# ultravideo/uvg266

Hardware: AMD Instinct MI355X
Metric: encoded fps (1080p all-intra --preset medium closed loop: CTU search with the reference's RD decisions -> deblock -> SAO -> slice data; Mpixels/s in config) (higher is better)
Workload: dtype u8

## Files before the change

### uvg266_amd/csrc/ctu_core.h

```cpp
#pragma once
#include <stdint.h>
#include <stddef.h>
#include <string.h>
#include "intra_pred_dev.h"
#if defined(__HIPCC__)
#include "satd_dev.h"
#endif
#include "vvc_tables.h"
#include "vvc_ctx_init.h"
#include "vvc_rdoq_tables.h"
#include "../../include/uvg266_hip.h"
#if defined(CTU_PB)
#include "inter_cand_dev.h"
#endif

#if defined(__HIPCC__)
#define CTU_NOINLINE __attribute__((noinline))
#define CTU_INLINE __attribute__((always_inline))
#define CTU_INLINE1 __attribute__((always_inline))
#define CTU_DEV static __device__
#define CTU_SHARED __shared__
#define CTU_TID ((int)(threadIdx.x & 63))
#define CTU_NT 64
#define CTU_WAVE (__builtin_amdgcn_readfirstlane((int)((threadIdx.x >> 6) - S->rot) & 3))
// ... 244 lines not shown
#if !defined(CTU_PB)
  int32_t req64, done64[2], m64[2];
  int32_t creq, cdone[2];
  struct { int32_t cu, cv, ssd_u, ssd_v, cy, ssd_y; double bits, bits_y; } h64[4];
#endif
  alignas(16) unsigned char arena[lds_cfg<PX>::slim ? (int)ARENA_BYTES_SLIM : (int)ARENA_BYTES];
#if defined(CTU_PB)
  pb_state pb;
  int32_t leaf_wave;
  double leaf_cost[4];
  double leaf_limit;
  int32_t depth_wave, skip_eval[4];
  pb_state pbx;
  alignas(16) unsigned char arena8[arena_bytes(8)];
  alignas(16) int16_t b8_tmp[6 * 2 * 120];
  PX b8_pred[6 * 64];
  int32_t b8_satd[8];
  pb_state pbx2;
  alignas(16) unsigned char arena16[arena_bytes(16)];
  alignas(16) PX cand64_px[6144];
  int16_t cand64_co[6144];
  uint32_t cur64[NMX];
#endif
};
#if defined(CTU_PB)
template <typename PX> constexpr size_t pb_lds_bytes(int waves) { return waves >= 4 ? sizeof(lds<PX>) : (waves == 3 ? offsetof(lds<PX>, pbx2) : offsetof(lds<PX>, pbx)); }
template <typename PX> CTU_DEV pb_state &pbq(lds<PX> *S) { const int r = CTU_WAVE; return r == 2 ? S->pbx : (r == 3 ? S->pbx2 : S->pb); }
#endif
template <typename PX> CTU_DEV wctx *wv_of(lds<PX> *S) { return &S->wv[S->vsel[CTU_WAVE]]; }

struct scratch {
  double cost_coeff[1024], cost_sig[1024], cost_coeff0[1024];
  uint16_t save_px[6144];
  int16_t save_co[6144];
  cu4 save_cu[256];
  int16_t cand_co[2016];
  uint16_t cand_px32[1536];
  int16_t lv32[1536];
  uint16_t scan_g[1024 + 256];
  uint32_t save_tree[512];
  uint16_t tree[256], mtt[256];
#if defined(CTU_PB)
  int32_t save_mot[256][8];
  uint8_t save_fl[256][8];
  int32_t pb_mot[17 * 17 + 1][8];
  uint8_t pb_fl[17 * 17][8];
  unsigned long long prof_pb[24];
#endif
  unsigned long long prof_lf[16];
  unsigned long long prof[4][32];
};

template <typename PX> struct job {
  params P;
  const PX *src_y, *src_u, *src_v;
  int src_stride, src_stride_c;
  PX *rec_y, *rec_u, *rec_v;
  int rec_stride, rec_stride_c;
  uvghip_scu_t *cu_tab;
  int cu_stride;
  int16_t *coeff;
  uint32_t *models_out;
  const uint32_t *models_in;
  scratch *W;
  int x, y;
#if defined(CTU_PB)
  const struct pb_job *pb;
  uint32_t *pbm_out;
  const uint32_t *pbm_in;
  int slice_type, init_qp;
#endif
};

template <typename PX> CTU_DEV CTU_GLB const PX *src_block(const job<PX> &J, int color, int bx, int by, int *pitch)
{
  const PX *p = color == 0 ? J.src_y : (color == 1 ? J.src_u : J.src_v);
  const int st = color == 0 ? J.src_stride : J.src_stride_c, sh = color != 0;
  *pitch = st;
  return (CTU_GLB const PX *)(p + (size_t)((J.y >> sh) + by) * st + (J.x >> sh) + bx);
}


CTU_DEV uint32_t *tab_ebits() { CTU_SHARED uint32_t t[512]; return t; }
CTU_DEV uint8_t *tab_rate() { CTU_SHARED uint8_t t[(NMX + 7) & ~7]; return t; }
CTU_DEV uint32_t *tab_rdoq_bits() { CTU_SHARED uint32_t t[2 * 244]; return t; }
#define kRate (tab_rate())

template <typename MP> CTU_DEV int m_state(MP m, int c) { return (int)(((m[c] & 0xffffu) + (m[c] >> 16)) >> 8); }
template <typename MP> CTU_DEV void m_update(MP m, int c, int bin)
{
  const int r0 = kRate[c] >> 4, r1 = kRate[c] & 15;
  uint32_t s0 = m[c] & 0xffffu, s1 = m[c] >> 16;
  s0 -= (s0 >> r0) & 0x7fe0u;
  s1 -= (s1 >> r1) & 0x7ffeu;
  if (bin) { s0 += (0x7fffu >> r0) & 0x7fe0u; s1 += (0x7fffu >> r1) & 0x7ffeu; }
  m[c] = (s0 & 0xffffu) | (s1 << 16);
}
template <typename MP> CTU_DEV double m_fbits(MP m, int c, int bin) { return (double)tab_ebits()[(m_state(m, c) << 1) ^ bin] / 32768.0; }
template <typename MP> CTU_DEV void m_code(MP m, int update, int c, int bin, double &bits)
{
  bits += m_fbits(m, c, bin);
  if (update) m_update(m, c, bin);
}

CTU_DEV void models_init_one(uint32_t *m, int i, int qp, int slice)
{
  const int v = k_ctx_init[slice][i];
  if (v == 255) { m[i] = 0; return; }
  const int slope = (v >> 3) - 4, offset = ((v & 7) * 18) + 1;
  int s = ((slope * (qp - 16)) >> 1) + offset;
  s = s < 1 ? 1 : (s > 127 ? 127 : s);
  const uint32_t p1 = (uint32_t)s << 8;
  m[i] = (p1 & 0x7fe0u) | ((p1 & 0x7ffeu) << 16);
}

CTU_DEV int scan_base(int log2n) { return log2n == 5 ? 0 : log2n == 4 ? 1024 : log2n == 3 ? 1280 : 1344; }
template <typename PX> CTU_DEV uint16_t *scan_of(lds<PX> *S, int log2n)
{
  if (lds_cfg<PX>::slim_scan) return log2n >= 4 ? S->scr->scan_g + (log2n == 5 ? 0 : 1024) : S->scan + (log2n == 3 ? 0 : 64);
  return S->scan + scan_base(log2n);
}
CTU_DEV int last_bits_off(int t, int log2n, int xy)
{
  const int cnt = 2 * log2n;
  const int base = log2n == 2 ? 0 : (log2n == 3 ? 8 : (log2n == 4 ? 20 : 36));
  return (t ? 56 : 0) + base + (xy ? cnt : 0);
}
CTU_DEV void diag_order(int n, uint8_t *out)
{
  int i = 0;
  for (int d = 0; d < 2 * n - 1; ++d)
    for (int x = 0; x <= d; ++x) {
      const int y = d - x;
      if (x < n && y < n) out[i++] = (uint8_t)(y * n + x);
    }
}
CTU_DEV int rdoq_diag_start(int n, int d)
{
  return d < n ? d * (d + 1) / 2 : n * n - (2 * n - 1 - d) * (2 * n - d) / 2;
}
template <typename PX> CTU_DEV void build_scans(lds<PX> *S)
{
  SERIAL {
    uint8_t in[16], cg[64];
    diag_order(4, in);
    for (int l2 = 2; l2 <= 5; ++l2) {
      const int n = 1 << l2, cgw = n >> 2;
      diag_order(cgw, cg);
      uint16_t *sc = scan_of(S, l2);
      if (l2 == 2) {
        for (int k = 0; k < 16; ++k) S->inv4[in[k]] = (uint8_t)k;
        for (int k = 0; k < 16; ++k) {
          const int x = in[k] & 3, y = in[k] >> 2;
          unsigned m = 0;
          if (x + 1 < 4) m |= 1u << S->inv4[y * 4 + x + 1];
          if (x + 2 < 4) m |= 1u << S->inv4[y * 4 + x + 2];
          if (y + 1 < 4) m |= 1u << S->inv4[(y + 1) * 4 + x];
          if (y + 2 < 4) m |= 1u << S->inv4[(y + 2) * 4 + x];
          if (x + 1 < 4 && y + 1 < 4) m |= 1u << S->inv4[(y + 1) * 4 + x + 1];
          S->deps4[k] = (uint16_t)m;
        }
      }
      for (int g = 0; g < cgw * cgw; ++g) {
        const int gx = cg[g] % cgw, gy = cg[g] / cgw;
        for (int k = 0; k < 16; ++k) sc[g * 16 + k] = (uint16_t)((gy * 4 + in[k] / 4) * n + gx * 4 + in[k] % 4);
      }
    }
  }
  CTU_SYNC();
}

CTU_DEV int16_t *lv_of(wctx *V, int color) { return color == 0 ? V->lv0 : (color == 1 ? V->lv1 : V->lv2); }
template <typename PX> CTU_DEV PX *plane(lds<PX> *S, int color) { return color == 0 ? S->Dy : (color == 1 ? S->Du : S->Dv); }
CTU_DEV int pitch_of(int color) { return color == 0 ? PY : PC; }
template <typename PX> CTU_DEV cu4 *cu_at(lds<PX> *S, int lx, int ly) { return &S->cu[((ly >> 2) + 1) * 17 + (lx >> 2) + 1]; }

template <typename PX> CTU_DEV int count_edge_cus(lds<PX> *S, int x, int y, int lx, int ly, int n, int left)
{
  if ((left && x == 0) || (!left && y == 0)) return 0;
  if (left && lx == 0) return (LCU - ly) / 4;
  if (!left && ly == 0) return n / 2;
  int amount = n & ~3;
  if (left) {
    if (ly == 0 && lx == 32 && cu_at(S, lx, ly)->log2 == 6) return 8;
    while (ly + amount < LCU && cu_at(S, lx - 4, ly + amount)->type != CU_NOTSET) amount += 4;
  } else {
    while (lx + amount < LCU && cu_at(S, lx + amount, ly - 4)->type != CU_NOTSET) amount += 4;
  }
  return (amount / 4) > (n / 4) ? amount / 4 : n / 4;
}

template <typename PX> CTU_NOINLINE CTU_DEV void build_refs(lds<PX> *S, const params &P, int color, int x, int y, int lx, int ly, int n, int cu_n)
{
  wctx *const V = wv_of(S);
  const int c = color != 0;
  const int w = n >> c;
  const int px_x = lx >> c, px_y = ly >> c;
  const int pit = pitch_of(color);
  const PX *D = plane(S, color) + (px_y + 1) * pit + px_x + 1;
  SERIAL {
    int al = count_edge_cus(S, x, y, lx, ly, n, 1) * (c ? 2 : 4);
    if (al > 2 * w) al = 2 * w;
    if (al > ((P.pic_h - y) >> c)) al = (P.pic_h - y) >> c;
    int at = count_edge_cus(S, x, y, lx, ly, n, 0) * (c ? 2 : 4);
    if (at > 2 * w) at = 2 * w;
    if (at > ((P.pic_w - x) >> c)) at = (P.pic_w - x) >> c;
    if (x > 0 && y > 0 && P.wpp && px_y == 0 && at > (LCU >> c) - px_x) at = (LCU >> c) - px_x;
    V->u_avail_left = al; V->u_avail_top = at;
  }
  CTU_SYNC();
  const int al = V->u_avail_left, at = V->u_avail_top;
  const int dc = 1 << (px_info<PX>::depth - 1);
  CTU_LDS uint16_t *const r_top = LDSP(uint16_t, V->top), *const r_left = LDSP(uint16_t, V->left);
  CTU_LDS uint16_t *const r_ftop = LDSP(uint16_t, V->ftop), *const r_fleft = LDSP(uint16_t, V->fleft);
  PAR_FOR(i, V->refn - 1) {
    int lv, tv;
    if (x > 0) lv = D[(i < al ? i : al - 1) * pit - 1];
    else lv = y > 0 ? D[-pit] : dc;
    if (y > 0) tv = D[-pit + (i < at ? i : at - 1)];
    else tv = x > 0 ? D[-1] : dc;
    r_left[i + 1] = (uint16_t)lv;
    r_top[i + 1] = (uint16_t)tv;
  }
  SERIAL {
    int corner;
    if (x > 0 && y > 0) corner = D[-pit - 1];
    else corner = x > 0 ? D[-1] : (y > 0 ? D[-pit] : dc);
    r_left[0] = r_top[0] = (uint16_t)corner;
  }
  CTU_SYNC();
  const int flim = 2 * (cu_n >> c) < V->refn - 1 ? 2 * (cu_n >> c) : V->refn - 1;
  PAR_FOR(i, V->refn) {
    int fl, ft;
    if (i == 0) fl = ft = (r_left[1] + 2 * r_left[0] + r_top[1] + 2) >> 2;
    else {
      fl = i < flim ? (r_left[i - 1] + 2 * r_left[i] + r_left[i + 1] + 2) >> 2 : r_left[i];
      ft = i < flim ? (r_top[i - 1] + 2 * r_top[i] + r_top[i + 1] + 2) >> 2 : r_top[i];
    }
    r_fleft[i] = (uint16_t)fl;
    r_ftop[i] = (uint16_t)ft;
  }
  CTU_SYNC();
}

template <typename PX> CTU_NOINLINE CTU_DEV void predict_block(lds<PX> *S, int mode, int color, int w, PX *dst_, int dp)
{
  wctx *const V = wv_of(S);
  const mode_info M = make_mode_info(mode, w, w, color != 0);
  const ref_rows_t<CTU_LDS const uint16_t *> R = {LDSP(const uint16_t, V->top), LDSP(const uint16_t, V->left), LDSP(const uint16_t, V->ftop), LDSP(const uint16_t, V->fleft)};
  const int dc = mode == 1 ? dc_value(R.top, R.left, w, w) : 0;
  typename mg_ptr<PX, PX>::type const dst = MGP(PX, PX, dst_);
  const int segs = w >> 2;
  PAR_FOR(t, w * segs) {
    const int yd = t / segs, xd0 = (t - yd * segs) * 4;
    int out[4];
    predict_row<4>(M, R, dc, color != 0, w, w, yd, xd0, (int)px_info<PX>::maxv, out);
    for (int i = 0; i < 4; ++i) {
      const int bx = M.vertical ? xd0 + i : yd, by = M.vertical ? yd : xd0 + i;
      dst[by * dp + bx] = (PX)out[i];
    }
  }
  CTU_SYNC();
}

CTU_DEV int iabs_(int v) { return v < 0 ? -v : v; }
CTU_DEV unsigned satd8_tile(int (&d)[64])
{
  for (int pass = 0; pass < 2; ++pass) {
    const int s = pass ? 8 : 1, t = pass ? 1 : 8;
    for (int l = 0; l < 8; ++l) {
      int *v = &d[l * t];
      for (int half = 4; half >= 1; half >>= 1)
        for (int base = 0; base < 8; base += 2 * half)
          for (int i = 0; i < half; ++i) {
            const int p = v[(base + i) * s], q = v[(base + i + half) * s];
            v[(base + i) * s] = p + q;
            v[(base + i + half) * s] = p - q;
          }
    }
  }
  unsigned sad = 0;
  for (int i = 0; i < 64; ++i) sad += (unsigned)iabs_(d[i]);
  sad -= (unsigned)iabs_(d[0]);
  sad += (unsigned)iabs_(d[0]) >> 2;
  return (sad + 2) >> 2;
}
CTU_DEV unsigned satd4_tile(int (&d)[16])
{
  for (int pass = 0; pass < 2; ++pass) {
    const int s = pass ? 4 : 1, t = pass ? 1 : 4;
    for (int l = 0; l < 4; ++l) {
      int *v = &d[l * t];
      const int a = v[0] + v[2 * s], b = v[0] - v[2 * s], c2 = v[s] + v[3 * s], e = v[s] - v[3 * s];
      v[0] = a + c2; v[s] = a - c2; v[2 * s] = b + e; v[3 * s] = b - e;
    }
  }
  unsigned satd = 0;
  for (int i = 0; i < 16; ++i) satd += (unsigned)iabs_(d[i]);
  satd -= (unsigned)iabs_(d[0]);
  satd += (unsigned)iabs_(d[0]) >> 2;
  return (satd + 1) >> 1;
}

template <typename PX> CTU_NOINLINE CTU_DEV void rough_costs(lds<PX> *S, const job<PX> &J, int lx, int ly, int n, const int32_t *modes, int n_modes)
{
  wctx *const V = wv_of(S);
  int sps;
  CTU_GLB const PX *Sy = src_block(J, 0, lx, ly, &sps);
  const int T = n >= 8 ? 8 : 4, tiles_x = n / T, tiles = tiles_x * tiles_x;
  const ref_rows_t<CTU_LDS const uint16_t *> R = {LDSP(const uint16_t, V->top), LDSP(const uint16_t, V->left), LDSP(const uint16_t, V->ftop), LDSP(const uint16_t, V->fleft)};
  const int dcv = dc_value(R.top, R.left, n, n);
  CTU_LDS uint32_t *const part = LDSP(uint32_t, V->part);
#if defined(__HIPCC__)
  const int n_flat = (n_modes > 0 && modes[0] < 2) + (n_modes > 1 && modes[1] < 2);
  for (int seg = 0; seg < 2; ++seg) {
  const int m_first = seg ? 0 : n_flat, total = (seg ? n_flat : n_modes - n_flat) * tiles * T;
  for (int base = 0; base < total; base += CTU_NT) {
    const int idx = base + CTU_TID;
    const bool on = idx < total;
    const int task0 = on ? idx / T : 0, r = idx & (T - 1);
    const int task = task0 + m_first * tiles;
    const int mi = task / tiles, tile = task - mi * tiles;
    const mode_info M = make_mode_info(modes[mi], n, n, 0);
    const int ty = tile / tiles_x, tx = tile - ty * tiles_x;
    int sad = 0, satd;
    if (T == 8) {
      int d[8], out[8];
      predict_row<8>(M, R, dcv, 0, n, n, ty * 8 + r, tx * 8, (int)px_info<PX>::maxv, out);
#pragma unroll
      for (int i = 0; i < 8; ++i) {
        const int wx = tx * 8 + i, wy = ty * 8 + r;
        const int bx = M.vertical ? wx : wy, by = M.vertical ? wy : wx;
        d[i] = on ? (int)Sy[by * sps + bx] - out[i] : 0;
        sad += iabs_(d[i]);
      }
      satd = satd8_cost(d, r);
      sad = dpp_group_sum<8>(sad);
    } else {
      int d[4], out[4];
      predict_row<4>(M, R, dcv, 0, n, n, r, 0, (int)px_info<PX>::maxv, out);
#pragma unroll
      for (int i = 0; i < 4; ++i) {
        const int bx = M.vertical ? i : r, by = M.vertical ? r : i;
        d[i] = on ? (int)Sy[by * sps + bx] - out[i] : 0;
        sad += iabs_(d[i]);
      }
      satd = satd4_cost(d, r);
      sad = dpp_group_sum<4>(sad);
    }
    if (on && r == 0) { part[2 * task] = (uint32_t)satd; part[2 * task + 1] = (uint32_t)sad; }
  }
  }
  CTU_SYNC();
#else
  PAR_FOR(task, n_modes * tiles) {
    const int mi = task / tiles, tile = task - mi * tiles;
    const int mode = modes[mi];
    const mode_info M = make_mode_info(mode, n, n, 0);
    const int ty = tile / tiles_x, tx = tile - ty * tiles_x;
    unsigned sad = 0, satd;
    if (T == 8) {
      int d[64];
      for (int r = 0; r < 8; ++r) {
        int out[8];
        predict_row<8>(M, R, dcv, 0, n, n, ty * 8 + r, tx * 8, (int)px_info<PX>::maxv, out);
        for (int i = 0; i < 8; ++i) {
          const int wx = tx * 8 + i, wy = ty * 8 + r;
          const int bx = M.vertical ? wx : wy, by = M.vertical ? wy : wx;
          const int df = (int)Sy[by * sps + bx] - out[i];
          d[r * 8 + i] = df;
          sad += (unsigned)iabs_(df);
        }
      }
      satd = satd8_tile(d);
    } else {
      int d[16];
      for (int r = 0; r < 4; ++r) {
        int out[4];
        predict_row<4>(M, R, dcv, 0, n, n, r, 0, (int)px_info<PX>::maxv, out);
        for (int i = 0; i < 4; ++i) {
          const int bx = M.vertical ? i : r, by = M.vertical ? r : i;
          const int df = (int)Sy[by * sps + bx] - out[i];
          d[r * 4 + i] = df;
          sad += (unsigned)iabs_(df);
        }
      }
      satd = satd4_tile(d);
    }
    part[2 * task] = satd;
    part[2 * task + 1] = sad;
  }
  CTU_SYNC();
#endif
}

#if defined(__HIPCC__)
CTU_DEV uint64_t rs_key(double c) { return (uint64_t)(uint32_t)__double2hiint(c) << 32 | (uint32_t)__double2loint(c); }
CTU_DEV uint32_t rs_wave_min(uint32_t v)
{
#define RS_MIN(x) { const uint32_t o = (uint32_t)(x); v = o < v ? o : v; }
  RS_MIN(__builtin_amdgcn_update_dpp(0, (int)v, 0xB1, 0xf, 0xf, true));
  RS_MIN(__builtin_amdgcn_update_dpp(0, (int)v, 0x4E, 0xf, 0xf, true));
  RS_MIN(__builtin_amdgcn_update_dpp(0, (int)v, 0x141, 0xf, 0xf, true));
  RS_MIN(__builtin_amdgcn_update_dpp(0, (int)v, 0x140, 0xf, 0xf, true));
  RS_MIN(__builtin_amdgcn_update_dpp((int)v, (int)v, 0x142, 0xa, 0xf, false));
  RS_MIN(__builtin_amdgcn_update_dpp((int)v, (int)v, 0x143, 0xc, 0xf, false));
#undef RS_MIN
  return (uint32_t)__builtin_amdgcn_readlane((int)v, 63);
}
struct rs_extra { bool on; uint64_t key; int seq, mode; };
struct rs_pick { int who; uint64_t key; };
CTU_DEV bool rs_key_lt(uint32_t khi, uint32_t klo, uint64_t k) { return ((uint64_t)khi << 32 | klo) < k; }
template <bool X> CTU_DEV rs_pick rs_pick_min(bool on, uint32_t khi, uint32_t klo, int seq, const rs_extra &x)
{
  const uint32_t none = 0xffffffffu;
  const uint32_t xh = (uint32_t)(x.key >> 32), xl = (uint32_t)x.key;
  const bool xon = X && x.on;
  rs_pick r;
  const unsigned long long b_on = __ballot(on);
  const int n_on = __popcll(b_on) + (xon ? 1 : 0);
  if (n_on == 0) { r.who = 0; r.key = ~0ull; return r; }
  uint32_t mh = 0;
  unsigned long long b1 = b_on;
  bool y = xon;
  if (n_on > 1) {
    mh = rs_wave_min(on ? khi : none);
    if (xon && xh < mh) mh = xh;
    b1 = __ballot(on && khi == mh);
    y = xon && xh == mh;
  }
  if (__popcll(b1) + (y ? 1 : 0) == 1) {
    if (y) { r.who = 64; r.key = x.key; }
    else {
      r.who = __builtin_ctzll(b1);
      r.key = (uint64_t)(uint32_t)__builtin_amdgcn_readlane((int)khi, r.who) << 32 | (uint32_t)__builtin_amdgcn_readlane((int)klo, r.who);
    }
    return r;
  }
  const bool t1 = on && khi == mh;
  uint32_t ml = rs_wave_min(t1 ? klo : none);
  if (y && xl < ml) ml = xl;
  const bool t2 = t1 && klo == ml, z = y && xl == ml;
  uint32_t ms = rs_wave_min(t2 ? (uint32_t)seq : none);
  r.key = (uint64_t)mh << 32 | ml;
  if (z && (uint32_t)x.seq < ms) r.who = 64;
  else {
    const unsigned long long w = __ballot(t2 && (uint32_t)seq == ms);
    r.who = w ? __builtin_ctzll(w) : 0;
  }
  return r;
}
struct rs_top3 { int m[3]; uint64_t k[3]; };
CTU_DEV void rs_insert(rs_top3 &B, int mode, uint64_t key)
{
  if (key < B.k[0]) { B.k[2] = B.k[1]; B.m[2] = B.m[1]; B.k[1] = B.k[0]; B.m[1] = B.m[0]; B.k[0] = key; B.m[0] = mode; }
  else if (key < B.k[1]) { B.k[2] = B.k[1]; B.m[2] = B.m[1]; B.k[1] = key; B.m[1] = mode; }
  else if (key < B.k[2]) { B.k[2] = key; B.m[2] = mode; }
}
template <bool X> CTU_DEV void rs_round(rs_top3 &B, bool on, uint32_t khi, uint32_t klo, int seq, int mode, rs_extra x)
{
  for (int i = 0; i < 3; ++i) {
    on = on && rs_key_lt(khi, klo, B.k[2]);
    if (X) x.on = x.on && x.key < B.k[2];
    const rs_pick pk = rs_pick_min<X>(on, khi, klo, seq, x);
    if (pk.key == ~0ull) break;
    rs_insert(B, pk.who < 64 ? __builtin_amdgcn_readlane(mode, pk.who) : x.mode, pk.key);
    on = on && CTU_TID != pk.who;
    if (X) x.on = x.on && pk.who != 64;
  }
}
#endif

CTU_DEV double count_bits(const int8_t *preds, double planar, double not_planar, double mpm_bit, double not_mpm_bit, int mode)
{
  int i = 0, smaller = 0;
  for (; i < 6; i++) {
    if (preds[i] == mode) break;
    if (mode > preds[i]) smaller += 1;
  }
  if (i == 0) return planar + mpm_bit;
  if (i < 6) return not_planar + mpm_bit + (i < 4 ? i : 4);
  return not_mpm_bit + 5 + (mode - smaller > 2);
}

CTU_DEV void dir_luma_predictor(int y, int8_t *preds, const cu4 *left_pu, const cu4 *above_pu)
{
  int left_dir = 0, above_dir = 0;
  if (left_pu && left_pu->type == CU_INTRA) left_dir = left_pu->mode;
  if (above_pu && above_pu->type == CU_INTRA && y % LCU != 0) above_dir = above_pu->mode;
  const int offset = 61, mod = 64;
  preds[0] = 0; preds[1] = 1; preds[2] = 50; preds[3] = 18; preds[4] = 46; preds[5] = 54;
  if (left_dir == above_dir) {
    if (left_dir > 1) {
      preds[0] = 0; preds[1] = (int8_t)left_dir;
      preds[2] = (int8_t)(((left_dir + offset) % mod) + 2); preds[3] = (int8_t)(((left_dir - 1) % mod) + 2);
      preds[4] = (int8_t)(((left_dir + offset - 1) % mod) + 2); preds[5] = (int8_t)((left_dir % mod) + 2);
    }
  } else if (left_dir > 1 && above_dir > 1) {
    preds[0] = 0; preds[1] = (int8_t)left_dir; preds[2] = (int8_t)above_dir;
    const int mx = preds[1] > preds[2] ? 1 : 2, mn = preds[1] > preds[2] ? 2 : 1;
    const int diff = preds[mx] - preds[mn];
    if (diff == 1) {
      preds[3] = (int8_t)(((preds[mn] + offset) % mod) + 2); preds[4] = (int8_t)(((preds[mx] - 1) % mod) + 2);
      preds[5] = (int8_t)(((preds[mn] + offset - 1) % mod) + 2);
    } else if (diff >= 62) {
      preds[3] = (int8_t)(((preds[mn] - 1) % mod) + 2); preds[4] = (int8_t)(((preds[mx] + offset) % mod) + 2);
      preds[5] = (int8_t)((preds[mn] % mod) + 2);
    } else if (diff == 2) {
      preds[3] = (int8_t)(((preds[mn] - 1) % mod) + 2); preds[4] = (int8_t)(((preds[mn] + offset) % mod) + 2);
      preds[5] = (int8_t)(((preds[mx] - 1) % mod) + 2);
    } else {
      preds[3] = (int8_t)(((preds[mn] + offset) % mod) + 2); preds[4] = (int8_t)(((preds[mn] - 1) % mod) + 2);
      preds[5] = (int8_t)(((preds[mx] + offset) % mod) + 2);
    }
  } else if (left_dir + above_dir >= 2) {
    preds[0] = 0;
    preds[1] = (int8_t)(left_dir < above_dir ? above_dir : left_dir);
    preds[2] = (int8_t)(((preds[1] + offset) % mod) + 2); preds[3] = (int8_t)(((preds[1] - 1) % mod) + 2);
    preds[4] = (int8_t)(((preds[1] + offset - 1) % mod) + 2); preds[5] = (int8_t)((preds[1] % mod) + 2);
  }
}
template <typename PX> CTU_DEV void mpm_neighbours(lds<PX> *S, int x, int y, int lx, int ly, int n, const cu4 **left, const cu4 **above)
{
  *left = x > 0 ? cu_at(S, lx - 1, ly + n - 1) : nullptr;
  *above = (ly > 0 && y > 0) ? cu_at(S, lx + n - 1, ly - 1) : nullptr;
}

#if defined(__HIPCC__)
template <typename PX> CTU_INLINE1 CTU_DEV void search_intra_rough(lds<PX> *S, const job<PX> &J, int x, int y, int lx, int ly, int n)
{
  wctx *const V = wv_of(S);
  const params &P = J.P;
  const int T = n >= 8 ? 8 : 4, tiles = (n / T) * (n / T);
  const int lane = CTU_TID;
  RQ_T0(J.W)
  SERIAL {
    const cu4 *l, *a;
    mpm_neighbours(S, x, y, lx, ly, n, &l, &a);
    dir_luma_predictor(y, V->mpm, l, a);
  }
  int offset = 1 << __builtin_amdgcn_readfirstlane(P.rough_levels);
  const int first_m = 2 + offset / 2;
  int nm = 2 + (66 - first_m) / offset + 1;
  if (lane < nm) V->rs_list[lane] = lane < 2 ? lane : first_m + (lane - 2) * offset;
  uint32_t pat = 1u << (first_m & (offset - 1));
  for (int sh = offset; sh < 32; sh <<= 1) pat |= pat << sh;
  uint32_t h0 = (pat & ~((1u << first_m) - 1u)) | 3u, h1 = pat, h2 = pat & 7u;
  CTU_SYNC();
  RQ_T(24);
  CTU_LDS const uint32_t *const mdl = LDSP(const uint32_t, V->cur), *const part = LDSP(const uint32_t, V->part);
  const double mpm_bit = m_fbits(mdl, M_MPM, 1), not_mpm_bit = m_fbits(mdl, M_MPM, 0);
  const double planar = m_fbits(mdl, M_PLANAR + 1, 0), not_planar = m_fbits(mdl, M_PLANAR + 1, 1);
  const rs_extra none = {false, 0, 0, 0};
  rs_top3 B = {{0, 0, 0}, {~0ull, ~0ull, ~0ull}};
  bool differs = false;
  for (int round = 0;; ++round) {
    rough_costs(S, J, lx, ly, n, V->rs_list, nm);
    RQ_T(25);
    bool on = lane < nm;
    int mode = 0;
    uint32_t khi = 0, klo = 0;
    if (on) {
      mode = V->rs_list[lane];
      unsigned satd = 0, sad = 0;
      for (int t = 0; t < tiles; ++t) { satd += part[2 * (lane * tiles + t)]; sad += part[2 * (lane * tiles + t) + 1]; }
      if (n >= 8) satd >>= (px_info<PX>::depth - 8);
      sad >>= (px_info<PX>::depth - 8);
      double c = (double)(satd < sad * 2 ? satd : sad * 2);
      c += count_bits(V->mpm, planar, not_planar, mpm_bit, not_mpm_bit, mode) * P.lambda_sqrt;
      khi = (uint32_t)__double2hiint(c); klo = (uint32_t)__double2loint(c);
    }
    RQ_T(26);
    const int seq = (round == 0 && lane < 2) ? 1 - lane : lane;
    if (round == 0)
      differs = __ballot(on && (khi != (uint32_t)__builtin_amdgcn_readlane((int)khi, 0) || klo != (uint32_t)__builtin_amdgcn_readlane((int)klo, 0))) != 0;
    rs_round<false>(B, on, khi, klo, seq, mode, none);
    offset >>= 1;
    if (!(offset > 0 && differs)) break;
    int tu[6];
#pragma unroll
    for (int j = 0; j < 6; ++j) {
      const int b = B.m[j >> 1], m = (j & 1) ? b + offset : b - offset;
      tu[j] = (b >= 3 && b <= 65 && m >= 2 && m <= 66) ? m : -1;
    }
    const int t = lane == 0 ? tu[0] : lane == 1 ? tu[1] : lane == 2 ? tu[2] : lane == 3 ? tu[3] : lane == 4 ? tu[4] : lane == 5 ? tu[5] : -1;
    bool listed = t >= 0 && !(((t < 32 ? h0 : (t < 64 ? h1 : h2)) >> (t & 31)) & 1u);
#pragma unroll
    for (int j = 0; j < 5; ++j) listed = listed && !(lane > j && tu[j] == t);
    const unsigned long long lm = __ballot(listed);
    if (listed) V->rs_list[__popcll(lm & ((1ull << lane) - 1ull))] = t;
    nm = __popcll(lm);
#pragma unroll
    for (int j = 0; j < 6; ++j)
      if (tu[j] >= 0) { const uint32_t bit = 1u << (tu[j] & 31); if (tu[j] < 32) h0 |= bit; else if (tu[j] < 64) h1 |= bit; else h2 |= bit; }
    CTU_SYNC();
    RQ_T(27);
  }
  SERIAL {
    V->u_mode = B.m[0];
    V->rs_cand[0] = __hiloint2double((int)(uint32_t)(B.k[0] >> 32), (int)(uint32_t)B.k[0]);
  }
  CTU_SYNC();
  RQ_T(27);
}
#else
template <typename PX> CTU_INLINE1 CTU_DEV void search_intra_rough(lds<PX> *S, const job<PX> &J, int x, int y, int lx, int ly, int n)
{
  wctx *const V = wv_of(S);
  const params &P = J.P;
  const int T = n >= 8 ? 8 : 4, tiles = (n / T) * (n / T);
  const cu4 *l, *a;
  mpm_neighbours(S, x, y, lx, ly, n, &l, &a);
  dir_luma_predictor(y, V->mpm, l, a);
  const double mpm_bit = m_fbits(V->cur, M_MPM, 1), not_mpm_bit = m_fbits(V->cur, M_MPM, 0);
  const double planar = m_fbits(V->cur, M_PLANAR + 1, 0), not_planar = m_fbits(V->cur, M_PLANAR + 1, 1);
  int offset = 1 << P.rough_levels;
  int32_t list[24];
  bool listed[67] = {};
  int nm = 0;
  list[nm++] = 0; list[nm++] = 1;
  for (int m = 2 + offset / 2; m <= 66; m += offset) list[nm++] = m;
  for (int i = 0; i < nm; ++i) listed[list[i]] = true;
  double best_cost[3] = {CTU_MAX_DOUBLE, CTU_MAX_DOUBLE, CTU_MAX_DOUBLE};
  int best_mode[3] = {0, 0, 0};
  bool differs = false;
  for (int round = 0;; ++round) {
    rough_costs(S, J, lx, ly, n, list, nm);
    double cost[24];
    for (int mi = 0; mi < nm; ++mi) {
      unsigned satd = 0, sad = 0;
      for (int t = 0; t < tiles; ++t) { satd += V->part[2 * (mi * tiles + t)]; sad += V->part[2 * (mi * tiles + t) + 1]; }
      if (n >= 8) satd >>= (px_info<PX>::depth - 8);
      sad >>= (px_info<PX>::depth - 8);
      cost[mi] = (double)(satd < sad * 2 ? satd : sad * 2) + count_bits(V->mpm, planar, not_planar, mpm_bit, not_mpm_bit, list[mi]) * P.lambda_sqrt;
      if (round == 0) differs = differs || cost[mi] != cost[0];
    }
    for (int i = 0; i < nm; ++i) {
      const int mi = (round == 0 && i < 2) ? 1 - i : i;
      for (int j = 0; j < 3; ++j)
        if (cost[mi] < best_cost[j]) {
          for (int k = 2; k > j; --k) { best_cost[k] = best_cost[k - 1]; best_mode[k] = best_mode[k - 1]; }
// ... 2229 lines not shown
```

### uvg266_amd/csrc/intra_pred_dev.h

```cpp
#pragma once
#include <stdint.h>
#include <stdlib.h>
#if !defined(__HIPCC__)
#ifndef __device__
#define __device__
#endif
#ifndef __forceinline__
#define __forceinline__ inline
#endif
static inline int clampi(int v, int lo, int hi) { return v < lo ? lo : (v > hi ? hi : v); }
static inline int min(int a, int b) { return a < b ? a : b; }
static inline int max(int a, int b) { return a > b ? a : b; }
static inline int __clz(int v) { return v ? __builtin_clz((unsigned)v) : 32; }
#endif

__device__ static const int16_t kSampleDisp[32] = {0, 1, 2, 3, 4, 6, 8, 10, 12, 14, 16, 18, 20, 23, 26, 29, 32, 35, 39, 45, 51,
                                                   57, 64, 73, 86, 102, 128, 171, 256, 341, 512, 1024};
__device__ static const int16_t kInvDisp[32] = {0, 16384, 8192, 5461, 4096, 2731, 2048, 1638, 1365, 1170, 1024, 910, 819, 712,
                                                630, 565, 512, 468, 420, 364, 321, 287, 256, 224, 191, 161, 128, 96, 64, 48, 32, 16};
__device__ static const int8_t kPreScale[32] = {8, 7, 6, 5, 5, 4, 4, 4, 3, 3, 3, 3, 3, 3, 2, 2, 2, 2, 2, 2, 1, 1, 1, 1, 1, 0, 0, 0,
                                                -1, -1, -2, -3};
__device__ static const int8_t kDistThres[8] = {24, 24, 24, 14, 2, 0, 0, 0};
__device__ static const int8_t kCubic[32][4] = {
  {0, 64, 0, 0},    {-1, 63, 2, 0},   {-2, 62, 4, 0},   {-2, 60, 7, -1},  {-2, 58, 10, -2}, {-3, 57, 12, -2},
  {-4, 56, 14, -2}, {-4, 55, 15, -2}, {-4, 54, 16, -2}, {-5, 53, 18, -2}, {-6, 52, 20, -2}, {-6, 49, 24, -3},
  {-6, 46, 28, -4}, {-5, 44, 29, -4}, {-4, 42, 30, -4}, {-4, 39, 33, -4}, {-4, 36, 36, -4}, {-4, 33, 39, -4},
  {-4, 30, 42, -4}, {-4, 29, 44, -5}, {-4, 28, 46, -6}, {-3, 24, 49, -6}, {-2, 20, 52, -6}, {-2, 18, 53, -5},
  {-2, 16, 54, -4}, {-2, 15, 55, -4}, {-2, 14, 56, -4}, {-2, 12, 57, -3}, {-2, 10, 58, -2}, {-1, 7, 60, -2},
  {0, 4, 62, -2},   {0, 2, 63, -1}};

__device__ __forceinline__ int ilog2_dev(int v) { return 31 - __clz(v); }

struct mode_info {
  int16_t mode;
  int16_t pred_mode;
  int8_t filtered;
  int8_t vertical;
  int16_t sample_disp;
  int16_t inv_disp;
  int8_t scale;
  int8_t use_cubic;
  int8_t pdpc;
  int8_t frac;
};

__device__ inline mode_info make_mode_info(int mode, int w, int h, int is_chroma)
{
  const int lw = ilog2_dev(w), lh = ilog2_dev(h);
  mode_info M;
  M.mode = (int16_t)mode;
  int pm = mode;
  if (lw != lh && mode > 1 && mode <= 66) {
    const int shift_tab[6] = {0, 6, 10, 12, 14, 15};
    const int d = abs(lw - lh);
    if (lw > lh && mode < 2 + shift_tab[d]) pm += 65;
    else if (lh > lw && mode > 66 - shift_tab[d]) pm -= 65;
  }
  M.pred_mode = (int16_t)pm;
  M.filtered = 0;
  M.vertical = 1; M.sample_disp = 0; M.inv_disp = 0; M.scale = 0; M.use_cubic = 1; M.pdpc = 0; M.frac = 0;
  if (mode >= 2) {
    const int d50 = abs(pm - 50), d18 = abs(pm - 18);
    const int dist = d50 < d18 ? d50 : d18;
    const int thres = kDistThres[(lw + lh) >> 1];
    const int vertical = pm >= 34;
    const int mode_disp = vertical ? pm - 50 : 18 - pm;
    const int amd = abs(mode_disp);
    const int sd = (mode_disp < 0 ? -1 : 1) * kSampleDisp[amd];
    if (!is_chroma && !(w == 4 && h == 4) && dist > thres) {
      const int sd8 = (int)(int8_t)sd;
      if ((abs(sd8) & 31) == 0) M.filtered = 1;
    }
    M.vertical = (int8_t)vertical;
    M.sample_disp = (int16_t)sd;
    M.inv_disp = kInvDisp[amd];
    const int side_log2 = vertical ? lh : lw;
    int scale = side_log2 - kPreScale[amd];
    if (scale > 2) scale = 2;
    M.scale = (int8_t)scale;
    M.frac = (abs(sd) & 31) != 0;
    M.use_cubic = !(dist > thres && M.frac);
    int pdpc = (w >= 4 && h >= 4);
    if (sd != 0) {
      if (pm > 1 && pm < 67) {
        if (mode_disp < 0) pdpc = 0;
        else if (mode_disp > 0) pdpc = pdpc && scale >= 0;
      }
    }
    M.pdpc = (int8_t)pdpc;
  } else if (mode == 0) {
    M.filtered = !is_chroma && !(w == 4 && h == 4) && (w * h > 32);
    M.pdpc = (w >= 4 && h >= 4);
  } else {
    M.pdpc = (w >= 4 && h >= 4);
  }
  return M;
}

template <typename RP> struct ref_rows_t {
  RP top, left, ftop, fleft;
};
typedef ref_rows_t<const uint16_t *> ref_rows;


template <typename RP> __device__ inline int dc_value(RP top, RP left, int w, int h)
{
  int sum = 0;
  if (w >= h) for (int i = 0; i < w; ++i) sum += top[1 + i];
  if (w <= h) for (int j = 0; j < h; ++j) sum += left[1 + j];
  const int denom = w == h ? w << 1 : max(w, h);
  return (sum + (denom >> 1)) >> ilog2_dev(denom);
}

template <int NP, typename RR>
__device__ __forceinline__ void predict_row(const mode_info &M, const RR &R, int dc, int is_chroma, int wd, int hd,
                                            int yd, int xd0, int maxv, int (&out)[NP])
{
  const auto top = M.filtered ? R.ftop : R.top;
  const auto left = M.filtered ? R.fleft : R.left;
  if (M.mode < 2) {
    const int lw = ilog2_dev(wd), lh = ilog2_dev(hd);
    const int scale = (lw + lh - 2) >> 2;
    const int sy = (yd << 1) >> scale, wt = 32 >> min(31, sy);
    const int l = left[yd + 1];
    if (M.mode == 0) {
      const int tr = top[wd + 1], bl = left[hd + 1];
      const int offset = 1 << (lw + lh), shift = 1 + lw + lh;
#pragma unroll
      for (int i = 0; i < NP; ++i) {
        const int x = xd0 + i, t = top[x + 1];
        const int hor = (l << lw) + (x + 1) * (tr - l);
        const int ver = (t << lh) + (yd + 1) * (bl - t);
        out[i] = ((hor << lh) + (ver << lw) + offset) >> shift;
      }
    } else {
#pragma unroll
      for (int i = 0; i < NP; ++i) out[i] = dc;
    }
    if (M.pdpc) {
#pragma unroll
      for (int i = 0; i < NP; ++i) {
        const int x = xd0 + i, sx = (x << 1) >> scale, wl = 32 >> min(31, sx);
        const int c = out[i];
        out[i] = c + ((wl * (l - c) + wt * ((int)top[x + 1] - c) + 32) >> 6);
      }
    }
    return;
  }
  const auto mainr = M.vertical ? top : left;
  const auto side = M.vertical ? left : top;
  const int sd = M.sample_disp;
  if (sd != 0) {
    const int inv = M.inv_disp;
    const int delta = sd * (yd + 1), di = delta >> 5, df = delta & 31;
    auto ref = [&](int idx) -> int {
      if (idx >= 0) return mainr[idx];
      int s = (-idx * inv + 256) >> 9;
      return side[min(s, hd)];
    };
    if (M.frac) {
      if (!is_chroma) {
        int f0, f1, f2, f3;
        if (M.use_cubic) { f0 = kCubic[df][0]; f1 = kCubic[df][1]; f2 = kCubic[df][2]; f3 = kCubic[df][3]; }
        else { f0 = 16 - (df >> 1); f1 = 32 - (df >> 1); f2 = 16 + (df >> 1); f3 = df >> 1; }
        int p[NP + 3];
#pragma unroll
        for (int k = 0; k < NP + 3; ++k) p[k] = ref(di + xd0 + k);
#pragma unroll
        for (int i = 0; i < NP; ++i)
          out[i] = clampi((f0 * p[i] + f1 * p[i + 1] + f2 * p[i + 2] + f3 * p[i + 3] + 32) >> 6, 0, maxv);
      } else {
#pragma unroll
        for (int i = 0; i < NP; ++i) {
          const int r1 = ref(xd0 + i + di + 1), r2 = ref(xd0 + i + di + 2);
          out[i] = r1 + ((df * (r2 - r1) + 16) >> 5);
        }
      }
    } else {
#pragma unroll
      for (int i = 0; i < NP; ++i) out[i] = ref(xd0 + i + di + 1);
    }
    if (M.pdpc) {
      const int scale = M.scale;
      const int lim = min(3 << scale, wd);
#pragma unroll
      for (int i = 0; i < NP; ++i) {
        const int x = xd0 + i;
        if (x < lim) {
          const int inv_sum = 256 + (x + 1) * inv;
          const int wl = 32 >> ((2 * x) >> scale);
          const int l = side[yd + (inv_sum >> 9) + 1];
          out[i] = out[i] + ((wl * (l - out[i]) + 32) >> 6);
        }
      }
    }
  } else {
    const int lw = ilog2_dev(wd), lh = ilog2_dev(hd);
    const int sc = (lw + lh - 2) >> 2;
    const int tl = mainr[0], l = side[1 + yd];
    const int lim = min(3 << sc, wd);
#pragma unroll
    for (int i = 0; i < NP; ++i) {
      const int x = xd0 + i;
      int v = mainr[1 + x];
      if (M.pdpc && x < lim) v = clampi(v + (((32 >> ((2 * x) >> sc)) * (l - tl) + 32) >> 6), 0, maxv);
      out[i] = v;
    }
  }
}
```

Measured before the change: 233.7.

## Specialize 8x8-tile rough intra cost path with branchless angular predictor

Adds a dedicated rough-cost routine for blocks of 8 and larger. Angular modes go through a branchless row predictor driven by packed LDS tables (displacement/inverse and cubic coefficients), with uniform scalars made wave-uniform via readfirstlane, and source samples are loaded before prediction. Planar/DC are handled separately, with the DC value computed by a wave-wide DPP reduction. This aims to cut divergent branches, integer divisions and per-mode setup overhead in the hot rough-cost search, at the risk of subtle prediction mismatches (PDPC, filter selection) and of relying on S->lf_disp/S->lf_cubic being initialised elsewhere.

```diff
diff --git a/uvg266_amd/csrc/ctu_core.h b/uvg266_amd/csrc/ctu_core.h
--- a/uvg266_amd/csrc/ctu_core.h
+++ b/uvg266_amd/csrc/ctu_core.h
@@ -570,12 +570,85 @@
   return (satd + 1) >> 1;
 }
 
+#if defined(__HIPCC__)
+CTU_DEV int rs_wave_sum(int v)
+{
+  v += dpp_xor1(v); v += dpp_xor2(v); v += dpp_mirror8(v); v += dpp_mirror16(v);
+  return __builtin_amdgcn_readlane(v, 0) + __builtin_amdgcn_readlane(v, 16) + __builtin_amdgcn_readlane(v, 32) + __builtin_amdgcn_readlane(v, 48);
+}
+template <typename PX> CTU_INLINE1 CTU_DEV void rough_costs8(lds<PX> *S, CTU_GLB const PX *Sy, int sps_, int n_, const int32_t *modes_, int n_modes_)
+{
+  wctx *const V = wv_of(S);
+  const int n = __builtin_amdgcn_readfirstlane(n_), n_modes = __builtin_amdgcn_readfirstlane(n_modes_), sps = __builtin_amdgcn_readfirstlane(sps_);
+  const int log2n = 31 - __builtin_clz((unsigned)n), lt = log2n - 3, lt2 = 2 * lt;
+  const int lane = CTU_TID, r = lane & 7, maxv = (int)px_info<PX>::maxv;
+  CTU_LDS const int32_t *const modes = LDSP(const int32_t, modes_);
+  CTU_LDS const uint32_t *const disp = LDSP(const uint32_t, S->lf_disp), *const cubic = LDSP(const uint32_t, S->lf_cubic);
+  const ref_rows_t<CTU_LDS const uint16_t *> R = {LDSP(const uint16_t, V->top), LDSP(const uint16_t, V->left), LDSP(const uint16_t, V->ftop), LDSP(const uint16_t, V->fleft)};
+  CTU_LDS uint32_t *const part = LDSP(uint32_t, V->part);
+  const int n_flat = __builtin_amdgcn_readfirstlane((n_modes > 0 && modes[0] < 2) + (n_modes > 1 && modes[1] < 2));
+  {
+    const int total = (n_modes - n_flat) << (lt2 + 3);
+    for (int base = 0; base < total; base += CTU_NT) {
+      const int idx = base + lane;
+      const bool on = idx < total;
+      const int task = (on ? idx >> 3 : 0) + (n_flat << lt2);
+      const int mi = task >> lt2, tile = task & ((1 << lt2) - 1), wy = (tile >> lt) * 8 + r, wx0 = (tile & ((1 << lt) - 1)) * 8;
+      const auto M = make_ang_mode(R, disp, modes[mi], log2n);
+      CTU_GLB const PX *const sp = Sy + (M.vertical ? wy * sps + wx0 : wx0 * sps + wy);
+      const int step = M.vertical ? 1 : sps;
+      int src[8], d[8], out[8], sad = 0;
+#pragma unroll
+      for (int i = 0; i < 8; ++i) src[i] = (int)sp[i * step];
+      ang_row8(M, cubic, n, wy, wx0, maxv, out);
+#pragma unroll
+      for (int i = 0; i < 8; ++i) {
+        d[i] = on ? src[i] - out[i] : 0;
+        sad += iabs_(d[i]);
+      }
+      const int satd = satd8_cost(d, r);
+      sad = dpp_group_sum<8>(sad);
+      if (on && r == 0) { part[2 * task] = (uint32_t)satd; part[2 * task + 1] = (uint32_t)sad; }
+    }
+  }
+  if (n_flat > 0) {
+    int acc = 0;
+    for (int i = lane; i < 2 * n; i += CTU_NT) acc += (int)*(i < n ? R.top + 1 + i : R.left + 1 + i - n);
+    const int dcv = (rs_wave_sum(acc) + n) >> (log2n + 1);
+    const int total = n_flat << (lt2 + 3);
+    for (int base = 0; base < total; base += CTU_NT) {
+      const int idx = base + lane;
+      const bool on = idx < total;
+      const int task = on ? idx >> 3 : 0;
+      const int mi = task >> lt2, tile = task & ((1 << lt2) - 1), wy = (tile >> lt) * 8 + r, wx0 = (tile & ((1 << lt) - 1)) * 8;
+      const mode_info M = make_mode_info(modes[mi] != 0, n, n, 0);
+      int src[8], d[8], out[8], sad = 0;
+#pragma unroll
+      for (int i = 0; i < 8; ++i) src[i] = (int)Sy[wy * sps + wx0 + i];
+      predict_row<8>(M, R, dcv, 0, n, n, wy, wx0, maxv, out);
+#pragma unroll
+      for (int i = 0; i < 8; ++i) {
+        d[i] = on ? src[i] - out[i] : 0;
+        sad += iabs_(d[i]);
+      }
+      const int satd = satd8_cost(d, r);
+      sad = dpp_group_sum<8>(sad);
+      if (on && r == 0) { part[2 * task] = (uint32_t)satd; part[2 * task + 1] = (uint32_t)sad; }
+    }
+  }
+  CTU_SYNC();
+}
+#endif
+
 template <typename PX> CTU_NOINLINE CTU_DEV void rough_costs(lds<PX> *S, const job<PX> &J, int lx, int ly, int n, const int32_t *modes, int n_modes)
 {
   wctx *const V = wv_of(S);
   int sps;
   CTU_GLB const PX *Sy = src_block(J, 0, lx, ly, &sps);
   const int T = n >= 8 ? 8 : 4, tiles_x = n / T, tiles = tiles_x * tiles_x;
+#if defined(__HIPCC__)
+  if (T == 8) { rough_costs8(S, Sy, sps, n, modes, n_modes); return; }
+#endif
   const ref_rows_t<CTU_LDS const uint16_t *> R = {LDSP(const uint16_t, V->top), LDSP(const uint16_t, V->left), LDSP(const uint16_t, V->ftop), LDSP(const uint16_t, V->fleft)};
   const int dcv = dc_value(R.top, R.left, n, n);
   CTU_LDS uint32_t *const part = LDSP(uint32_t, V->part);
@@ -588,23 +661,10 @@
     const bool on = idx < total;
     const int task0 = on ? idx / T : 0, r = idx & (T - 1);
     const int task = task0 + m_first * tiles;
-    const int mi = task / tiles, tile = task - mi * tiles;
+    const int mi = task / tiles;
     const mode_info M = make_mode_info(modes[mi], n, n, 0);
-    const int ty = tile / tiles_x, tx = tile - ty * tiles_x;
     int sad = 0, satd;
-    if (T == 8) {
-      int d[8], out[8];
-      predict_row<8>(M, R, dcv, 0, n, n, ty * 8 + r, tx * 8, (int)px_info<PX>::maxv, out);
-#pragma unroll
-      for (int i = 0; i < 8; ++i) {
-        const int wx = tx * 8 + i, wy = ty * 8 + r;
-        const int bx = M.vertical ? wx : wy, by = M.vertical ? wy : wx;
-        d[i] = on ? (int)Sy[by * sps + bx] - out[i] : 0;
-        sad += iabs_(d[i]);
-      }
-      satd = satd8_cost(d, r);
-      sad = dpp_group_sum<8>(sad);
-    } else {
+    {
       int d[4], out[4];
       predict_row<4>(M, R, dcv, 0, n, n, r, 0, (int)px_info<PX>::maxv, out);
 #pragma unroll
diff --git a/uvg266_amd/csrc/intra_pred_dev.h b/uvg266_amd/csrc/intra_pred_dev.h
--- a/uvg266_amd/csrc/intra_pred_dev.h
+++ b/uvg266_amd/csrc/intra_pred_dev.h
@@ -208,3 +208,72 @@
     }
   }
 }
+
+template <typename RP> struct ang_mode {
+  RP mainr, side;
+  int sd, inv;
+  int sc, lim;
+  bool vertical, cubic;
+};
+template <typename RR, typename TP>
+__device__ __forceinline__ auto make_ang_mode(const RR &R, TP disp, int mode, int log2n) -> ang_mode<decltype(R.top)>
+{
+  ang_mode<decltype(R.top)> M;
+  const int thres = log2n <= 3 ? 14 : (log2n == 4 ? 2 : 0);
+  M.vertical = mode >= 34;
+  const int md = M.vertical ? mode - 50 : 18 - mode, amd = md < 0 ? -md : md;
+  const uint32_t t = disp[amd];
+  const int asd = (int)(t & 0xff);
+  M.inv = (int)(t >> 8);
+  M.sd = md < 0 ? -asd : asd;
+  const bool far = amd > thres, frac = (asd & 31) != 0;
+  const bool filtered = far && !frac;
+  M.cubic = !(far && frac);
+  const auto top = filtered ? R.ftop : R.top;
+  const auto left = filtered ? R.fleft : R.left;
+  M.mainr = M.vertical ? top : left;
+  M.side = M.vertical ? left : top;
+  int sc = log2n - (23 - __clz(3 * M.inv - 2));
+  sc = sc > 2 ? 2 : sc;
+  sc = md == 0 ? (2 * log2n - 2) >> 2 : sc;
+  const bool pd = md >= 0 && sc >= 0;
+  M.sc = pd ? sc : 0;
+  M.lim = pd ? min(3 << M.sc, 1 << log2n) : 0;
+  return M;
+}
+template <typename AM, typename TP>
+__device__ __forceinline__ void ang_row8(const AM &M, TP cubic_tab, int n, int yd, int xd0, int maxv, int (&out)[8])
+{
+  const int delta = M.sd * (yd + 1), di = delta >> 5, df = delta & 31;
+  int p[11];
+  int proj = 256 - (di + xd0) * M.inv;
+#pragma unroll
+  for (int k = 0; k < 11; ++k) {
+    const int idx = di + xd0 + k;
+    const int s = min(proj >> 9, n);
+    const auto q = idx >= 0 ? M.mainr + idx : M.side + s;
+    p[k] = *q;
+    proj -= M.inv;
+  }
+  const int h = df >> 1;
+  const uint32_t fc = (uint32_t)cubic_tab[df];
+  const uint32_t f = M.cubic ? fc : 0x00102010u + (uint32_t)h * 0x0100FEFFu;
+  const int f0 = (int)(int8_t)(f & 0xff), f1 = (int)(int8_t)((f >> 8) & 0xff), f2 = (int)(int8_t)((f >> 16) & 0xff), f3 = (int)(int8_t)(f >> 24);
+#pragma unroll
+  for (int i = 0; i < 8; ++i) out[i] = clampi((f0 * p[i] + f1 * p[i + 1] + f2 * p[i + 2] + f3 * p[i + 3] + 32) >> 6, 0, maxv);
+  if (xd0 < M.lim) {
+    const int tl = M.mainr[0];
+    const bool pure = M.sd == 0;
+    int acc = 256 + (xd0 + 1) * M.inv;
+#pragma unroll
+    for (int i = 0; i < 8; ++i) {
+      const int x = xd0 + i;
+      const bool in = x < M.lim;
+      const int l = M.side[in ? yd + (acc >> 9) + 1 : 0];
+      const int wl = 32 >> ((2 * x) >> M.sc);
+      const int v = clampi(out[i] + ((wl * (l - (pure ? tl : out[i])) + 32) >> 6), 0, maxv);
+      out[i] = in ? v : out[i];
+      acc += M.inv;
+    }
+  }
+}
```

Result: faster. 250.7, median of 6 (+7.3%).
